# zhizdev/sparsefusion

Measured on AMD Instinct MI355X. Metric: novel views/sec, distillation steps (2 NGP renders fwd+bwd + VAE enc/dec + 51-eval PLMS + LPIPS), 256^2 / 32x32 latents, 2-view synthetic hydrant, higher is better.
Workload: dtype bf16 MFMA operands / f32 accumulate (UNet); f32 (NGP render)

## Files before the change

### include/sparsefusion_hip.h

```cpp
#ifndef SPARSEFUSION_HIP_H
#define SPARSEFUSION_HIP_H

#include <stdint.h>

#ifdef __cplusplus
extern "C" {
#endif

#define SF_OK 0
#define SF_ERR_INVALID 1
#define SF_ERR_LAUNCH 2

const char* sf_last_error(void);
int sf_abi_version(void);
int sf_operand_is_f16(void);


int sf_grid_encode_forward(const float* inputs, const float* embeddings,
                           const int32_t* offsets, float* outputs,
                           uint32_t B, uint32_t D, uint32_t C, uint32_t L,
                           float S, uint32_t H, float* dy_dx,
                           uint32_t gridtype, int align_corners,
                           const int32_t* h_offsets, void* stream);

// ... 174 lines not shown
  uint32_t n_tensors;
  float beta1, beta2, eps;
  float bias_correction2_sqrt;
  float one_minus_beta1, one_minus_beta2;
} sf_adam_args;
int sf_adam_multi(const sf_adam_args* args, void* stream);

uint32_t sf_loss_partial_rows(void);
int sf_upsample2x_forward(const float* in, float* out, uint32_t planes, uint32_t h, uint32_t w, void* stream);
int sf_upsample2x_backward(const float* grad_out, float* grad_in, uint32_t planes, uint32_t h, uint32_t w, void* stream);
int sf_render_loss_forward(const float* img, const float* sil, const float* target_rgb, const float* target_mask, uint64_t n_img,
                           uint64_t n_sil, float scaling, float* partial, void* stream);
int sf_render_loss_backward(const float* img, const float* sil, const float* target_rgb, const float* target_mask, uint64_t n_img,
                            uint64_t n_sil, float scaling, float c_rgb, float c_sil, float c_opacity, float c_entropy,
                            const float* grad_loss, float* grad_img, float* grad_sil, void* stream);
int sf_fusion_loss_forward(const float* img, const float* pred, const float* view_weight, const float* sil, uint32_t views,
                           uint64_t per_view_img, uint64_t per_view_sil, float* partial, void* stream);
int sf_fusion_loss_backward(const float* img, const float* pred, const float* view_weight, const float* sil, uint32_t views,
                            uint64_t per_view_img, uint64_t per_view_sil, float c_l1, float c_opacity, float c_entropy,
                            const float* grad_loss, float* grad_img, float* grad_sil, void* stream);

int sf_plan_run(const sf_op* ops, uint32_t n_ops, void* stream);
uint64_t sf_conv_igemm_t_launches(void);
int sf_plan_profile(const sf_op* ops, uint32_t n_ops, void* stream, float* h_ms);

uint64_t sf_conv_packed_elems(uint32_t Cout, uint32_t cin_pad, uint32_t kh, uint32_t kw);
int sf_conv_pack_weights(const float* h_w, uint32_t Cout, uint32_t Cin,
                         uint32_t cin_pad, uint32_t kh, uint32_t kw,
                         uint16_t* h_out);

int sf_plms_update(const float* x, const float* eps, const float* noise,
                   const float* h_coef6, uint64_t n, float* x_prev, float* x0,
                   void* stream);
int sf_plms_combine(const float* e0, const float* e1, const float* e2,
                    const float* e3, const float* h_c4, uint64_t n, float* out,
                    float* keep_e0, void* stream);
int sf_plms_step(const float* e0, const float* e1, const float* e2, const float* e3,
                 const float* h_c4, float* keep_e0, const float* x, const float* noise,
                 const float* h_coef6, uint64_t n, float* x_prev,
                 const float* row_src, float* row_dst, uint64_t row_n, void* stream);

#ifdef __cplusplus
}
#endif
#endif
```

### sparsefusion_amd/_lib.py

```python
import ctypes as C
import os

import torch

_HERE = os.path.dirname(os.path.abspath(__file__))
_DEFAULT_LIB = "libsparsefusion_hip_f16.so" if os.environ.get("SF_OPERAND", "bf16").lower() in ("f16", "fp16", "half") else "libsparsefusion_hip.so"
LIB_PATH = os.environ.get("SF_HIP_LIB") or os.path.join(_HERE, _DEFAULT_LIB)

_lib = None

c_f32p = C.c_void_p
c_i32p = C.c_void_p
u32 = C.c_uint32
u64 = C.c_uint64


class SfNgpField(C.Structure):
    _fields_ = [("embeddings", C.c_void_p), ("h_offsets", C.c_void_p), ("L", u32), ("S", C.c_float),
                ("H", u32), ("gridtype", u32),
                ("w0", C.c_void_p), ("b0", C.c_void_p), ("w1", C.c_void_p), ("b1", C.c_void_p),
                ("w2", C.c_void_p), ("b2", C.c_void_p), ("bound", C.c_float)]


class SfNgpFieldGrad(C.Structure):
# ... 54 lines not shown
    "sf_fusion_loss_forward": (C.c_int, [c_f32p, c_f32p, c_f32p, c_f32p, u32, u64, u64, c_f32p, C.c_void_p]),
    "sf_fusion_loss_backward": (C.c_int, [c_f32p, c_f32p, c_f32p, c_f32p, u32, u64, u64, C.c_float, C.c_float, C.c_float,
                                          c_f32p, c_f32p, c_f32p, C.c_void_p]),
    "sf_ngp_density": (C.c_int, [C.POINTER(SfNgpField), c_f32p, u32, c_f32p, c_f32p, C.c_void_p]),
    "sf_ngp_density_lattice": (C.c_int, [C.POINTER(SfNgpField), c_f32p, c_f32p, c_f32p, u32, u32, u32, c_f32p, C.c_void_p]),
    "sf_gaussian3d_workspace_bytes": (u64, [u32, u32, u32]),
    "sf_gaussian3d": (C.c_int, [c_f32p, c_f32p, u32, u32, u32, C.c_float, C.c_float, C.c_void_p, C.c_void_p, u64, C.c_void_p]),
    "sf_mc_workspace_bytes": (u64, [u32, u32, u32]),
    "sf_mc_count": (C.c_int, [c_f32p, u32, u32, u32, C.c_float, C.c_void_p, u64, C.c_void_p, C.c_void_p]),
    "sf_mc_emit": (C.c_int, [c_f32p, u32, u32, u32, C.c_float, C.c_void_p, u64, c_f32p, c_i32p, C.c_void_p]),
    "sf_ngp_render_forward": (C.c_int, [C.POINTER(SfNgpField), c_f32p, c_f32p, c_f32p, u32, u32, C.c_float,
                                        c_f32p, c_f32p, c_f32p, u32, C.c_float, c_f32p, c_f32p, c_f32p, c_f32p,
                                        c_f32p, c_f32p, c_f32p, c_f32p, c_f32p, c_f32p, u64, C.c_void_p]),
    "sf_ngp_render_backward": (C.c_int, [C.POINTER(SfNgpField), C.POINTER(SfNgpFieldGrad), c_f32p, c_f32p,
                                         c_f32p, u32, u32, c_f32p, c_f32p, c_f32p, c_f32p, c_f32p,
                                         C.c_float, c_f32p, c_f32p, u32, c_f32p, c_f32p, u64, C.c_void_p]),
    "sf_ngp_render_workspace_bytes": (u64, [u32, u32]),
    "sf_ngp_render_forward_workspace_bytes": (u64, [u32, u32]),
    "sf_ngp_render_cache_bytes": (u64, [u32, u32]),
    "sf_ngp_render_occ_eval": (C.c_int, [C.POINTER(SfNgpField), c_f32p, c_f32p, c_f32p, c_f32p, C.c_void_p, C.c_float, u32, u32, u32,
                                         c_f32p, C.c_float, u32, c_f32p, c_f32p, c_f32p, C.c_void_p]),
    "sf_plan_run": (C.c_int, [C.POINTER(SfOp), u32, C.c_void_p]),
    "sf_conv_igemm_t_launches": (u64, []),
    "sf_plan_profile": (C.c_int, [C.POINTER(SfOp), u32, C.c_void_p, C.c_void_p]),
    "sf_conv_packed_elems": (u64, [u32, u32, u32, u32]),
    "sf_conv_pack_weights": (C.c_int, [C.c_void_p, u32, u32, u32, u32, u32, C.c_void_p]),
    "sf_plms_update": (C.c_int, [c_f32p, c_f32p, c_f32p, C.c_void_p, u64, c_f32p, c_f32p, C.c_void_p]),
    "sf_plms_combine": (C.c_int, [c_f32p, c_f32p, c_f32p, c_f32p, C.c_void_p, u64, c_f32p, c_f32p, C.c_void_p]),
    "sf_plms_step": (C.c_int, [c_f32p, c_f32p, c_f32p, c_f32p, C.c_void_p, c_f32p, c_f32p, c_f32p, C.c_void_p, u64, c_f32p, c_f32p, c_f32p, u64, C.c_void_p]),
}


_handles = {}


def _load(path):
    if path not in _handles:
        if not os.path.exists(path):
            raise RuntimeError(
                f"{path} is missing: build it with `python -m sparsefusion_amd.build` (`--f16` for the IEEE-half operand build; "
                "there is no CPU fallback for the sparsefusion_amd hot path)")
        handle = C.CDLL(path)
        for name, (res, args) in SIGNATURES.items():
            fn = getattr(handle, name)
            fn.restype = res
            fn.argtypes = args
# ... 40 lines not shown
```

### sparsefusion_amd/csrc/conv_igemm_t.h

```cpp
#pragma once
#include "sf_dev.h"
#include "conv_lds.h"

#define SF_IGT_SPLITK 0
#define SF_IGT_PIXSHUF 1

#define SF_IGEMM_T_VARIANTS(X) \
  X(5, 256, 256, 4, 2, 1, 0, 2, 2, 4, 1, 0) \
  X(4, 256, 512, 4, 2, 1, 0, 1, 2, 8, 1, 0) \
  X(3, 512, 1024, 4, 2, 1, 0, 1, 1, 4, 1, 0) \
  X(2, 1024, 4096, 1, 1, 0, 0, 1, 1, 1, 1, 1) \
  X(3, 1024, 2048, 1, 1, 0, 0, 1, 1, 1, 1, 1) \
  X(4, 512, 1024, 1, 1, 0, 0, 1, 2, 1, 1, 1) \
  X(5, 256, 4, 3, 1, 1, 0, 1, 1, 4, 1, 0)

constexpr int sf_igt_log2(int v) { return v <= 1 ? 0 : 1 + sf_igt_log2(v >> 1); }

#ifndef SF_IGT_KNOCKOUT
#define SF_IGT_KNOCKOUT 0
#endif

template <int HL, int CIN, int COUT, int K, int STRIDE, int PAD, int UPS, int WM, int WN, int GROUPS, bool A_FP32, int EPI>
SF_KERNEL(256) void k_conv_igemm_t(ConvArgs a) {
  constexpr int H = 1 << HL, HO = (H + 2 * PAD - K) / STRIDE + 1, HOL = sf_igt_log2(HO), M = HO * HO;
  constexpr int CCH = CIN / 32, CCL = sf_igt_log2(CCH), KS = K * K * CCH, NF = (COUT + 15) / 16, NPAD = NF * 16;
  constexpr int MT = M / 16 / WM, NT = NF / WN, SPW = (KS + GROUPS * 4 - 1) / (GROUPS * 4);
  constexpr bool RAGGED = SPW * GROUPS * 4 != KS;
  constexpr int STEP_REGS = WM * (A_FP32 ? 8 : 4) + WN * 4;
  constexpr int D = SPW * STEP_REGS <= 96 ? SPW : (96 / STEP_REGS < 2 ? 2 : 96 / STEP_REGS);
  constexpr int LDC = COUT / 4;
  static_assert((1 << HOL) == HO && (1 << CCL) == CCH && CIN % 32 == 0, "k_conv_igemm_t: power-of-two map and channel chunks");
  static_assert(M % (16 * WM) == 0 && NF % WN == 0, "k_conv_igemm_t: the tiles divide the output evenly (no clamped fragments)");
  static_assert(EPI == SF_IGT_SPLITK ? GROUPS > 1 : (GROUPS == 1 && COUT % 64 == 0 && M % 16 == 0), "k_conv_igemm_t: epilogue kind");
  static_assert(H * H * CIN < (1 << 28) && NF * KS * 64 < (1 << 27) && GROUPS * M * NPAD < (1 << 29), "k_conv_igemm_t: 32-bit offsets");

  sf_touch_kernarg<(int)sizeof(ConvArgs)>();
  SF_SHARED __attribute__((aligned(16))) float red[3][WM * WN * 4 * 64];
  const int lane = threadIdx.x & 63, wave = sf_uniform((int)(threadIdx.x >> 6));
  const int tile = blockIdx.x % (MT * NT), grp = blockIdx.x / (MT * NT);
  const int nt = tile % NT, mt = tile / NT;
  const int k0 = (grp * 4 + wave) * SPW;
  const int cgrp = (lane >> 4) * 8;

  float bq[WN];
#pragma unroll
  for (int ni = 0; ni < WN; ++ni) bq[ni] = EPI == SF_IGT_PIXSHUF ? a.bias[(nt * WN + ni) * 16 + (lane & 15)] : 0.0f;

  int py[WM], px[WM];
#pragma unroll
  for (int mi = 0; mi < WM; ++mi) {
    const int m = (mt * WM + mi) * 16 + (lane & 15);
    py[mi] = (m >> HOL) * STRIDE - PAD;
    px[mi] = (m & (HO - 1)) * STRIDE - PAD;
  }
  const float* in32 = reinterpret_cast<const float*>(a.in);
  const sf_opnd* in16 = reinterpret_cast<const sf_opnd*>(a.in);
// ... 70 lines not shown
        for (int r = 0; r < 4; ++r) red[wave - 1][((mi * WN + ni) * 4 + r) * 64 + lane] = acc[mi][ni][r];
  }
  sf_sync();
  if (wave != 0) return;
#pragma unroll
  for (int mi = 0; mi < WM; ++mi)
#pragma unroll
    for (int ni = 0; ni < WN; ++ni)
#pragma unroll
      for (int r = 0; r < 4; ++r) {
        const int idx = ((mi * WN + ni) * 4 + r) * 64 + lane;
        acc[mi][ni][r] += red[0][idx] + red[1][idx] + red[2][idx];
      }
  if (SF_IGT_KNOCKOUT == 3) {
#ifndef SF_HOST_EMU
#pragma unroll
    for (int mi = 0; mi < WM; ++mi)
#pragma unroll
      for (int ni = 0; ni < WN; ++ni) asm volatile("" ::"v"(acc[mi][ni]), "v"(bq[ni]));
#endif
    return;
  }

#pragma unroll
  for (int mi = 0; mi < WM; ++mi) {
#pragma unroll
    for (int ni = 0; ni < WN; ++ni) {
      const int nf = nt * WN + ni;
      const int n = nf * 16 + (lane & 15);
      const int m0 = (mt * WM + mi) * 16 + (lane >> 4) * 4;
      if (EPI == SF_IGT_SPLITK) {
#pragma unroll
        for (int r = 0; r < 4; ++r) a.ws[(grp * M + m0 + r) * NPAD + n] = acc[mi][ni][r];
      } else {
        float bv = bq[ni];
        SF_USE_FROM_HERE(bv);
        float v[4], sm = 0.0f, sq = 0.0f;
#pragma unroll
        for (int r = 0; r < 4; ++r) {
          v[r] = sf_silu(acc[mi][ni][r] + bv);
          sm += v[r];
          sq = fmaf(v[r], v[r], sq);
        }
        sm = sf_wave_sum(sm);
        sq = sf_wave_sum(sq);
        if (lane == 0) {
          float* sl = a.slots_out + (((mt * WM + mi) * 4 + (nf & 3)) * (LDC >> 4) + (nf >> 2)) * 2;
          sl[0] = sm;
          sl[1] = sq;
        }
        const int c = n >> 2, ii = (n >> 1) & 1, jj = n & 1;
#pragma unroll
        for (int r = 0; r < 4; ++r) {
          const int m = m0 + r, oy = m >> HOL, ox = m & (HO - 1);
          a.out[((2 * oy + ii) * (2 * HO) + 2 * ox + jj) * LDC + c] = v[r];
        }
      }
    }
  }
}
```

### sparsefusion_amd/csrc/initx.hip

```cpp
#include "sf_common.h"
#include "initx.h"

int sf_plan_initx_op(const sf_op* op, void* stream) {
  InitXArgs a;
  a.x = (const float*)op->p[0]; a.base = (const float*)op->p[1]; a.w = (const ix_bf16x8*)op->p[2]; a.out = (float*)op->p[3];
  a.slots = (float*)op->p[4];
  a.B = op->i[0]; a.H = op->i[1]; a.W = op->i[2]; a.Cx = op->i[3]; a.ld = op->i[4];
  for (int k = 0; k < 3; ++k) { a.cw[k] = op->i[5 + k]; a.co[k] = op->i[8 + k]; a.woff[k] = op->i[11 + k]; }
  if (!a.x || !a.base || !a.w || !a.out || a.B < 1) SF_FAIL(SF_ERR_INVALID, "init_x: missing operand");
  if (a.H % IX_TILE || a.W % IX_TILE || a.Cx < 1 || a.Cx > 4) SF_FAIL(SF_ERR_INVALID, "init_x: H, W multiples of 8 and 1..4 latent channels");
  if ((a.cw[0] != 64 && a.cw[0] != 128) || (a.cw[1] != 32 && a.cw[1] != 64) || (a.cw[2] != 32 && a.cw[2] != 64))
    SF_FAIL(SF_ERR_INVALID, "init_x: channel slices (%d, %d, %d) not instantiated", a.cw[0], a.cw[1], a.cw[2]);
  if (a.slots && (a.ld % 16 || a.co[0] % 16 || a.co[1] % 16 || a.co[2] % 16)) SF_FAIL(SF_ERR_INVALID, "init_x: slots need 16-aligned channel slices");
  const uint32_t grid = (uint32_t)a.B * (a.H / IX_TILE) * (a.W / IX_TILE) * 3;
  k_init_x<<<grid, 256, 0, (hipStream_t)stream>>>(a);
  SF_CHECK_LAUNCH("init_x");
  return SF_OK;
}
```

### sparsefusion_amd/csrc/unet_ops.hip

```cpp

#include "sf_common.h"
#include "plan_ops.h"
#include "sf_dev.h"
#include "gemm_rows.h"
#include "conv_halo.h"
#include "conv_halo_small.h"
#include "conv_igemm.h"
#include "conv_igemm_t.h"
#include "attn_ln.h"
#include <math.h>

typedef __attribute__((ext_vector_type(8))) sf_opnd bf16x8;
typedef __attribute__((ext_vector_type(4))) sf_opnd bf16x4;
typedef __attribute__((ext_vector_type(4))) float f32x4;
typedef __attribute__((address_space(1))) float gfloat;

__device__ __forceinline__ void atomic_add_f32(float* p, float v) {
  (void)__builtin_amdgcn_global_atomic_fadd_f32((gfloat*)p, v);
}
__device__ __forceinline__ float silu_f(float v) { return v / (1.0f + __expf(-v)); }
__device__ __forceinline__ float sigmoid_f(float v) { return 1.0f / (1.0f + __expf(-v)); }
__device__ __forceinline__ float gelu_f(float v) { return 0.5f * v * (1.0f + erff(v * 0.70710678118654752f)); }

__device__ __forceinline__ float wave_sum(float v) {
// ... 402 lines not shown
  for (long i = blockIdx.x * 256L + threadIdx.x; i < n; i += (long)gridDim.x * 256) out[i] += a[i];
}

__global__ void k_time_emb(const float* __restrict__ t, const float* __restrict__ w, float* __restrict__ out, int B,
                           int half) {
  const int i = blockIdx.x * blockDim.x + threadIdx.x;
  if (i >= B * half) return;
  const int b = i / half, j = i - b * half;
  const float fr = t[b] * w[j] * 2.0f * 3.14159265358979323846f;
  float* o = out + (long)b * (1 + 2 * half);
  if (j == 0) o[0] = t[b];
  o[1 + j] = sinf(fr);
  o[1 + half + j] = cosf(fr);
}

template <int WM, int WN>
static void launch_conv(const ConvArgs& a, bool a_fp32, int blocks, hipStream_t st) {
  if (a_fp32) k_conv_igemm<WM, WN, true><<<blocks, 256, 0, st>>>(a);
  else k_conv_igemm<WM, WN, false><<<blocks, 256, 0, st>>>(a);
}

static unsigned long long g_igemm_t_launches = 0;
extern "C" uint64_t sf_conv_igemm_t_launches(void) { return g_igemm_t_launches; }
static bool launch_conv_t(const ConvArgs& a, int WM, int WN, bool a_fp32, int blocks, hipStream_t st) {
  if (a.B != 1 || a.H != a.W || a.kh != a.kw || a.accum || a.resid || a.relu || a.co_off) return false;
  const int epi = a.pixshuf ? SF_IGT_PIXSHUF : SF_IGT_SPLITK;
  if (a.pixshuf ? (!a.slots_out || !a.bias || a.ldc * 4 != a.Cout || a.groups != 1) : (a.groups < 2 || !a.ws)) return false;
#define SF_TRY_IGT(hl_, cin_, cout_, k_, s_, p_, ups_, wm_, wn_, g_, f32_, epi_) \
  if (a.H == (1 << hl_) && a.Cin == cin_ && a.Cout == cout_ && a.kh == k_ && a.stride == s_ && a.pad == p_ && a.ups == ups_ && WM == wm_ && \
      WN == wn_ && a.groups == g_ && a_fp32 == (bool)f32_ && epi == epi_ && a.Ho == ((1 << hl_) + 2 * p_ - k_) / s_ + 1 && a.Wo == a.Ho) { \
    k_conv_igemm_t<hl_, cin_, cout_, k_, s_, p_, ups_, wm_, wn_, g_, (bool)f32_, epi_><<<blocks, 256, 0, st>>>(a); \
    ++g_igemm_t_launches; \
    return true; \
  }
  SF_IGEMM_T_VARIANTS(SF_TRY_IGT)
#undef SF_TRY_IGT
  return false;
}

static int conv_glds_depth() { return 4; }
template <int BNF, int NST, bool GN>
static int launch_conv_glds(const ConvArgs& a, int nblk, double* part, int cg, hipStream_t st) {
  static unsigned mask = 0;
  const uint32_t lds = conv_glds_lds_bytes(BNF, NST);
  int dev = 0;
  if (hipGetDevice(&dev) != hipSuccess) SF_FAIL(SF_ERR_LAUNCH, "hipGetDevice failed");
  if (dev >= 32 || !(mask & (1u << dev))) {
    if (hipFuncSetAttribute(reinterpret_cast<const void*>(&k_conv_glds<BNF, NST, GN>), hipFuncAttributeMaxDynamicSharedMemorySize, (int)lds) != hipSuccess)
      SF_FAIL(SF_ERR_LAUNCH, "hipFuncSetAttribute(max dynamic LDS) failed");
    if (dev < 32) mask |= 1u << dev;
  }
  k_conv_glds<BNF, NST, GN><<<nblk, 512, lds, st>>>(a, part, cg);
  SF_CHECK_LAUNCH("conv_glds");
  return SF_OK;
// ... 126 lines not shown
      } else if (bnf == 4) {
        if (f32) k_conv_lds_gn<4, true><<<nblk, 256, 0, st>>>(a, part, cg); else k_conv_lds_gn<4, false><<<nblk, 256, 0, st>>>(a, part, cg);
      } else {
        SF_FAIL(SF_ERR_INVALID, "conv: unsupported LDS tile %d", bnf);
      }
      SF_CHECK_LAUNCH("conv_lds_gn");
      return SF_OK;
    }
    if (halo) return bnf == 8 ? launch_conv_halo_nst<8, false>(a, nblk, nullptr, 0, halo, st) : launch_conv_halo_nst<4, false>(a, nblk, nullptr, 0, halo, st);
    if (glds) {
      if (int rc = bnf == 8 ? launch_conv_glds_nst<8, false>(a, nblk, nullptr, 0, glds, st) : launch_conv_glds_nst<4, false>(a, nblk, nullptr, 0, glds, st)) return rc;
      return conv_splitk_tail(op, a, M, st);
    }
    if (bnf == 8) {
      if (f32) k_conv_lds<8, true><<<nblk, 256, 0, st>>>(a); else k_conv_lds<8, false><<<nblk, 256, 0, st>>>(a);
    } else if (bnf == 4) {
      if (f32) k_conv_lds<4, true><<<nblk, 256, 0, st>>>(a); else k_conv_lds<4, false><<<nblk, 256, 0, st>>>(a);
    } else {
      SF_FAIL(SF_ERR_INVALID, "conv: unsupported LDS tile %d", bnf);
    }
    SF_CHECK_LAUNCH("conv_lds");
    return conv_splitk_tail(op, a, M, st);
  }
  if ((op.flags & 512) && launch_conv_t(a, WM, WN, f32, blocks, st)) {
    SF_CHECK_LAUNCH("conv_igemm_t");
    return conv_splitk_tail(op, a, M, st);
  }
  switch (tile) {
    case 1 * 16 + 1: launch_conv<1, 1>(a, f32, blocks, st); break;
    case 1 * 16 + 2: launch_conv<1, 2>(a, f32, blocks, st); break;
    case 1 * 16 + 4: launch_conv<1, 4>(a, f32, blocks, st); break;
    case 2 * 16 + 1: launch_conv<2, 1>(a, f32, blocks, st); break;
    case 2 * 16 + 2: launch_conv<2, 2>(a, f32, blocks, st); break;
    case 2 * 16 + 4: launch_conv<2, 4>(a, f32, blocks, st); break;
    case 4 * 16 + 1: launch_conv<4, 1>(a, f32, blocks, st); break;
    case 4 * 16 + 2: launch_conv<4, 2>(a, f32, blocks, st); break;
    case 4 * 16 + 4: launch_conv<4, 4>(a, f32, blocks, st); break;
    default: SF_FAIL(SF_ERR_INVALID, "conv: unsupported wave tile %dx%d", WM, WN);
  }
  SF_CHECK_LAUNCH("conv_igemm");
  return conv_splitk_tail(op, a, M, st);
}

static int lazy_from_op(const sf_op& op, int ibase, int M, LazySrc& lz) {
  lz.mode = op.i[ibase]; lz.groups = op.i[ibase + 1]; lz.npad = op.i[ibase + 2]; lz.M = M;
  lz.a = (const float*)op.p[8]; lz.b = (const float*)op.p[9]; lz.r = (const float*)op.p[10];
  if (lz.mode < 0 || lz.mode > 2) SF_FAIL(SF_ERR_INVALID, "lazy source: unknown mode %d", lz.mode);
// ... 419 lines not shown
```

### sparsefusion_amd/plan.py

```python
import torch

from . import _lib

OP_CONV, OP_GN_ACT, OP_LN, OP_GEMV, OP_ATTN, OP_GCA_POOL, OP_ELTWISE, OP_MEMSET, OP_TIME_EMB, OP_SPLITK_REDUCE = range(1, 11)
OP_FCONV, OP_SLOTS, OP_GCA, OP_INITX, OP_GN_FINALIZE = 14, 15, 16, 17, 18
FNORM_NONE, FNORM_GN_SELF, FNORM_GN_SLOTS, FNORM_LN, FNORM_ATTN = range(5)
LDS_MAX = 163840
SKIP_SCALE = 2 ** -0.5


class _Arena:

    def __init__(self, nbytes=None, device=None):
        self.off = 0
        self.buf = torch.empty(nbytes, dtype=torch.uint8, device=device) if nbytes else None

    def alloc(self, nbytes):
        nbytes = (nbytes + 255) // 256 * 256
        off = self.off
        self.off += nbytes
        return (self.buf.data_ptr() + off) if self.buf is not None else (1 << 20) + off


class _T:
    __slots__ = ("ptr", "rows", "C", "HW", "lazy", "slots", "writer", "twin")

    def __init__(self, ptr, rows, C, HW=None):
        self.ptr, self.rows, self.C, self.HW = ptr, rows, C, HW
        self.lazy = None
        self.slots = None
        self.twin = None
        self.writer = None


class PlanOwner:
    conv_waves_target = 1024
    lds_conv_min_blocks = 0
    lds_mid_min_rows = 0
    lds_mid_min_batch = 8
    gn_epilogue = False
    gn_one = True
    ln_wave = True
    tb_stride = 0
    lazy_consumers = 0
    ss_total = 0
    igemm_t = 0
    igemm_t_variants = ()
    tile_override = None

    def conv_tiling(self, m_frags, n_frags, KS, pixshuf=False):
        ov = self.tile_override
        if ov and (m_frags, n_frags, KS, bool(pixshuf)) in ov:
            return ov[(m_frags, n_frags, KS, bool(pixshuf))]
        best = None
        mfma = m_frags * n_frags * KS
        w_bytes = n_frags * KS * 1024
        for WM in (1, 2, 4):
            if m_frags % WM or (m_frags <= 4 and WM != m_frags and m_frags in (1, 2, 4)):
                continue
            for WN in (1, 2, 4):
                if n_frags % WN:
                    continue
                tiles = (m_frags // WM) * (n_frags // WN)
                for groups in ((1,) if pixshuf else (1, 2, 4, 8, 16, 32)):
                    if groups > 1 and KS // (4 * groups) < 2:
                        continue
                    waves = tiles * groups * 4
                    util = min(1.0, waves / self.conv_waves_target)
                    t_hbm = w_bytes / 4.0e12 / util
# ... 118 lines not shown
                tile, groups = 256 + bnf, 1
                if twin is not None and ldc == Cout and co_off == 0:
                    twin_ws = twin.ptr
            elif mid and M >= mid:
                glds_ok = not x_f32 and x.C % 64 == 0 and Cout % 4 == 0 and ldc % 4 == 0 and co_off % 4 == 0
                stages = KS // 2 if glds_ok else (KS + 1) // 2
                g = 1 if pixshuf else max(1, min(256 // blocks, stages // 4, 16))
                if glds_ok and k == 3 and stride == 1 and pad == 1 and H == W and H in (4, 8) and not pixshuf:
                    g = max(1, min(256 // blocks, x.C // 128, 16))
                tile, groups = 256 + bnf, g
        ws, wi = 0, 0
        if groups > 1:
            wi = self.acquire_ws(groups * M * n_frags * 16 * 4)
            ws = self.ws_ptrs[wi]
        elif twin_ws:
            ws = twin_ws
        defer = bool(defer and not relu and not gelu and 1 < groups <= defer_max_groups and not accum and not pixshuf and co_off == 0 and ldc == Cout == out.C and M == out.rows
                     and (self.u.lazy_consumers & 1))
        bias, res = self.wptr(bname) if bname else 0, resid.ptr if resid else 0
        slots = 0
        if want_slots and pixshuf and tile < 256 and (Cout // 4) % 16 == 0 and ldc % 16 == 0 and co_off % 16 == 0 and (Ho * Wo) % 16 == 0 and not accum:
            slots = self.misc.alloc(4 * M // 16 * (ldc // 16) * 2 * 4)
        nchw = bool(nchw and groups > 1 and not defer and not accum and not resid and tile < 256 and co_off == 0 and ldc == Cout)
        igt = False
        if self.u.igemm_t and tile < 256 and B == 1 and H == W and (Ho, Wo) == ((H + 2 * pad - k) // stride + 1,) * 2 and not (accum or res or relu or gelu or co_off):
            key = (H.bit_length() - 1, x.C, Cout, k, stride, pad, int(bool(upsampled)), WM, WN, groups, int(bool(x_f32)), 1 if pixshuf else 0)
            if key in self.u.igemm_t_variants and H == 1 << key[0] and (self.u.igemm_t >> self.u.igemm_t_variants.index(key)) & 1:
                igt = bool(slots and bias and ldc * 4 == Cout) if pixshuf else groups > 1
        self.op(OP_CONV, (1 if x_f32 else 0) | (2 if pixshuf else 0) | (4 if accum else 0) | (8 if defer else 0) |
                (16 if upsampled else 0) | (32 if relu else 0) | (64 if gelu else 0) | (256 if nchw else 0) | (512 if igt else 0),
                p=(x.ptr, w_ptr if w_ptr is not None else self.wptr(wname), bias, out.ptr, res, ws, 0, slots),
                i=(B, H, W, x.C, Ho, Wo, Cout, ldc, co_off, k, k, stride, pad, groups, tile))
        if defer:
            out.lazy = ("splitk", ws, bias, res, groups, n_frags * 16, wi)
            self.ws_owners[wi] = out
        out.slots = slots or None
        self.last_conv_nchw = nchw
        out.writer = self.ops[-1] if (tile >= 256 and co_off == 0 and ldc == Cout == out.C and M == out.rows) else None
        out.twin = twin if (twin is not None and tile >= 256 and groups == 1 and ws == twin.ptr) else None
        return Ho, Wo

    def gn_act(self, x, skip, gname, ss_ptr, out, raw=None, silu=True, groups=8, eps=1e-5):
        C1, C2 = x.C, (skip.C if skip else 0)
        self.need(skip)
        lp, li = self.take_lazy(x, ("splitk", "gate"))
        stats = self.zero.alloc(self.B * groups * 2 * 8)
        ready = 0
        wr = x.writer
        cg = (C1 // groups) if not skip else 0
        if (self.u.gn_epilogue and wr is not None and not (wr.flags & 128) and li[0] == 0 and cg in (4, 8, 16)
                and x.HW and x.HW % 128 == 0 and x.rows == self.B * x.HW):
            part = self.misc.alloc(x.rows // 128 * groups * 2 * 8)
            wr.flags |= 128
# ... 43 lines not shown
```

### sparsefusion_amd/unet.py

```python
import math
import os

import numpy as np
import torch
import torch.nn as nn

from . import _lib
from .plan import (FNORM_ATTN, FNORM_GN_SELF, FNORM_GN_SLOTS, FNORM_LN, FNORM_NONE, LDS_MAX, OP_ATTN, OP_CONV, OP_ELTWISE, OP_FCONV, OP_GCA,
                   OP_GCA_POOL, OP_GEMV, OP_GN_ACT, OP_GN_FINALIZE, OP_INITX, OP_LN, OP_MEMSET, OP_SLOTS, OP_SPLITK_REDUCE, OP_TIME_EMB,
                   SKIP_SCALE, Plan, PlanOwner, _T)

PAIR_TILES = {(1, 1, 1), (1, 1, 2), (1, 2, 2), (2, 2, 2), (4, 2, 2)}
PIPE_TILES = {(1, 1, 4), (1, 2, 4), (1, 1, 6), (1, 2, 6), (2, 1, 6), (2, 2, 6), (2, 1, 8), (2, 2, 8), (2, 1, 12), (2, 2, 12), (4, 1, 16), (4, 2, 16)}
CONV3S_VARIANTS = {(5, 256, 5, 2, 2), (5, 256, 3, 2, 2), (4, 256, 4, 1, 1), (4, 256, 2, 1, 1), (4, 512, 4, 1, 2), (4, 512, 2, 1, 2),
                   (3, 512, 3, 1, 1), (3, 1024, 3, 1, 1), (5, 256, 5, 4, 2), (5, 256, 3, 4, 2),
                   (4, 256, 2, 2, 1), (4, 256, 2, 2, 2), (4, 512, 2, 2, 2), (3, 512, 3, 2, 1), (3, 1024, 3, 2, 1), (3, 1024, 3, 2, 2)}
CONV3S_RC_VARIANTS = {(5, 256, 256, 256, 3, 2, 2), (4, 512, 256, 512, 2, 1, 2), (3, 1024, 512, 1024, 3, 1, 1)}
IGEMM_T_VARIANTS = ((5, 256, 256, 4, 2, 1, 0, 2, 2, 4, 1, 0), (4, 256, 512, 4, 2, 1, 0, 1, 2, 8, 1, 0), (3, 512, 1024, 4, 2, 1, 0, 1, 1, 4, 1, 0),
                    (2, 1024, 4096, 1, 1, 0, 0, 1, 1, 1, 1, 1), (3, 1024, 2048, 1, 1, 0, 0, 1, 1, 1, 1, 1), (4, 512, 1024, 1, 1, 0, 0, 1, 2, 1, 1, 1),
                    (5, 256, 4, 3, 1, 1, 0, 1, 1, 4, 1, 0))
ATTN_LDS_BYTES = 8 * 16 * 36 * 4 + 2 * 8 * 4 * 68 * 4
TILE_PICKS = {(4, 32, 128, False): (1, 2, 8),
              (4, 128, 32, True): (1, 1, 1),
              (16, 64, 16, True): (1, 2, 1),
              (64, 1, 72, False): (1, 1, 4),
              (64, 16, 128, False): (2, 4, 4), (16, 32, 128, False): (1, 4, 4), (4, 64, 256, False): (1, 2, 4),
              (4, 64, 288, False): (1, 4, 4), (4, 256, 32, True): (1, 2, 1), (16, 128, 32, True): (1, 4, 1),
              (64, 64, 16, True): (1, 2, 1)}

SWITCHES = (
    ("conv_waves_target", 1024, "waves wanted per conv launch (4 per CU) before split-K stops"),
    ("lds_conv_min_blocks", 96, "use k_conv_lds when a layer has at least this many 128 x 128 output tiles"),
    ("lds_mid_min_rows", 128, "r06: convs of >= this many rows that have too few 128-row tiles for lds_conv_min_blocks run on the LDS-tiled kernels with split-K groups (Plan.conv); 0 = off"),
    ("igemm_t", 127, "the one-of-a-kind implicit GEMMs of the B = 1 eval on k_conv_igemm_t (compile-time geometry, csrc/conv_igemm_t.h; op flag 512): bit j = row j of IGEMM_T_VARIANTS; 0: k_conv_igemm"),
    ("merged_down_conv4", True, "r06: the merged 3x3 + 1x1 conv of the last Downsample on k_conv4_gn<64, 0, false> at B = 1; False: k_conv_igemm"),
    ("rc_small_tiles", 32, "r06: bit mask of map sides (32 | 16 | 8) whose B >= 2 (conv1 || res_conv) pairs keep the B = 1 tile of k_conv3s_rc (32: B = 2 eval 1.155 -> 1.139 ms, B = 4 1.562 -> 1.520; 32 | 16: B = 4 1.580, B = 8 2.451 -> 2.550)"),
    ("gn_one", True, "r06: GroupNorm passes of B >= 32 plans (B * 8 >= 256 workgroups) in one launch (k_gn_one); False: k_gn_stats + k_gn_apply everywhere"),
    ("lds_mid_min_batch", 8, "... in plans of at least this many images (the B = 1 .. 4 plans keep their measured kernels)"),
    ("unfused_min_rows_4", 256, "r06: 4x4-level ResnetBlocks with B*16 >= this leave the fused kernels (as unfused_min_rows at 32x32 / 16x16; measured: B = 8 loses 0.12 ms, B = 16 gains 0.22, B = 32 0.49); 0 = never"),
    ("unfused_min_rows_8", 1024, "... 8x8 level (k_conv3_halo_sm; measured: B = 8 loses 0.14 ms, B = 16 gains 0.04, B = 32 0.56)"),
    ("unfused_lin_min_rows", 256, "r06: attention / feed-forward linears of the 4x4 level with >= this many token rows leave the fused kernels (measured: B = 16 3.683 -> 3.670 ms, B = 32 4.664 -> 4.472)"),
    ("unfused_min_rows_16", 4096, "r06: the 16x16 level's own threshold (0 = unfused_min_rows; measured with k_gemm_rows_ks / the r06 plans: B = 16 3.641 -> 3.313 ms; 2048 rows lose: B = 8 2.454 -> 2.512)"),
    ("unfused_min_rows_32", 0, "... 32x32 level (4096 rows lose: B = 4 1.575 -> 1.686 ms)"),
    ("unfused_min_rows", 8192, "ResnetBlocks with B*H*W >= this at the 32x32 / 16x16 levels leave the fused kernels (_Plan.resnet; measured r03: B = 8 eval 3.33 -> 2.96 ms, B = 32 11.5 -> 7.8 ms, B = 4 unchanged)"),
    ("lazy_consumers", 3, "bit 0: split-K reductions, bit 1: gated residuals are materialised by their first consumer"),
    ("fused", True, "GroupNorm inside the conv launches (k_conv_fused) wherever the layer fits; False = the first-round plan"),
    ("pair_res_conv", True, "conv1 || res_conv of a ResnetBlock in one launch"),
    ("res_conv_beside_pool", True, "4x4 gca blocks: the res_conv shares the GlobalContext pooling launch instead"),
    ("initx_direct", True, "latent half of the init conv as one direct-convolution launch"),
    ("big_tile_min_batch", 2, "batch from which the 8x8 / 16x16 / 32x32 maps use 32- / 32- / 64-pixel tiles (r03: B = 2 eval 1.70 -> 1.50 ms, B = 4 2.62 -> 2.02, B = 32 16.4 -> 11.5; at B = 1 they would leave half the CUs idle; 999 = never)"),
    ("gca_epilogue_pool", True, "GlobalContext pooling in conv2's epilogue (False = k_gca_pool launch)"),
    ("fconv_pipe", True, "slot-GroupNorm 3x3 convs on k_conv_fused_pipe (staging || matrix work)"),
    ("producer_slots", True, "r04: k_init_x / the Upsample epilogue leave their consumers' statistics slots, the final conv's split-K reduction writes NCHW (False: the r03 k_slots / k_unpack_out launches; parity tests)"),
    ("attn_in_out_proj", True, "the 16-token attention core in the prologue of its output projection (False: k_attn16 launch; parity tests)"),
    ("ln_wave", True, "r05: LayerNorm of <= 256 rows of 512 | 1024 | 2048 channels on k_layernorm_wave (False: op flag 4 = k_layernorm)"),
    ("gate_t", True, "r05: GlobalContext gate with a compile-time hidden width (k_gca_gate_t; False: k_gca_gate)"),
    ("conv4_reduce_min_batch", 4, "r05: from this batch on a 4x4 split-K conv1 is reduced by its own launch instead of by conv2's gather (0 = never)"),
# ... 631 lines not shown
        self.x_in, self.t_in = self.f32(B, u.channels * HW), self.f32(B, 1)
        self.cond_in = self.f32(B, u.cond_images_channels * HW)
        self.tb = self.f32(B, u.tb_stride)
        self.ss = self.tb
        self.emit_time(B, self.tb.ptr, self.t_in.ptr)
        self.n_time_ops = len(self.ops)
        self.op(OP_MEMSET, 0, p=(self.zero.buf.data_ptr() if self.zero.buf is not None else 1,), i=(0,))
        memset_op = self.ops[-1]
        xin = self.f32(B * HW, cpad, HW)
        self.op(OP_ELTWISE, 2, p=(self.cond_in.ptr, self.x_in.ptr, 0, xin.ptr), i=(B, HW, u.cond_images_channels, u.channels, cpad))
        x = self.f32(B * HW, u.dim, HW)
        co = 0
        for i, k in enumerate((3, 7, 15)):
            cw = u.spec_shapes[f"init_conv.convs.{i}.weight"][0]
            self.conv(xin, True, R, R, f"init_conv.convs.{i}.weight", f"init_conv.convs.{i}.bias", x, u.dim, co, cw, k, 1, k // 2)
            co += cw
        self.n_init_ops = len(self.ops)
        self.x0, self.base = x, self.f32(B * HW, u.dim, HW)
        full_ops, full_written, self.ops, self.written = self.ops, self.written, [], set()
        cws = [u.spec_shapes[f"init_conv.convs.{i}.weight"][0] for i in range(3)]
        if (u.initx_direct and u.fused and R % 8 == 0 and u.channels <= 4 and cws[0] in (64, 128)
                and cws[1] in (32, 64) and cws[2] in (32, 64) and "__init_xw__" in self.w):
            offs, woffs = [0, cws[0], cws[0] + cws[1]], u.initx_woffs
            self.op(OP_INITX, 0, p=(self.x_in.ptr, self.base.ptr, self.wptr("__init_xw__"), x.ptr),
                    i=(B, R, R, u.channels, u.dim, cws[0], cws[1], cws[2], offs[0], offs[1], offs[2], woffs[0], woffs[1], woffs[2]))
        else:
            xin_x = self.f32(B * HW, 32, HW)
            self.op(OP_ELTWISE, 2, p=(self.x_in.ptr, self.x_in.ptr, 0, xin_x.ptr), i=(B, HW, 0, u.channels, 32))
            co = 0
            for i, k in enumerate((3, 7, 15)):
                cw = cws[i]
                self.conv(xin_x, True, R, R, f"__init_x__.{i}", None, x, u.dim, co, cw, k, 1, k // 2, resid=self.base)
                co += cw
        self.init_x_ops, self.ops, self.written = self.ops, full_ops, full_written
        hiddens = []
        H = R
        n_lv = len(u.in_out)
        for lv, (di, do) in enumerate(u.in_out):
            x = self.resnet(f"downs.{lv}.1", x, None, di, H)
            for r in range(u.nres[lv]):
                x = self.resnet(f"downs.{lv}.2.{r}", x, None, di, H, gca=True)
                hiddens.append(x)
            if u.attns[lv]:
                x = self.transformer(f"downs.{lv}.3", x)
            hiddens.append(x)
            if lv < n_lv - 1:
                y = self.f32(B * (H // 2) ** 2, do, (H // 2) ** 2)
# ... 443 lines not shown
```

Measured before the change: 17.76.

## Add compile-time-geometry init_x kernel and optional LDS-transposed pixel-shuffle epilogue

Adds k_init_x_t, a specialised kernel for the B = 1 sampler's latent init convolution (3/7/15 kernels) with weights preloaded into registers and one m-fragment per workgroup. It is enabled by default through a new op flag. It also adds an optional PIXLDS path that stages the pixel-shuffle epilogue of k_conv_igemm_t through LDS so the output goes out as vector stores; that path is off by default (pixshuf_lds = 0). The cost targeted is a small part of each UNet eval, so the effect on the whole distillation step is limited, and the heavier register use of the new kernel could lower occupancy.

New measurement: 17.83, median of 6. About the same (+0.4%).

```diff
diff --git a/include/sparsefusion_hip.h b/include/sparsefusion_hip.h
--- a/include/sparsefusion_hip.h
+++ b/include/sparsefusion_hip.h
@@ -220,6 +220,8 @@
 
 int sf_plan_run(const sf_op* ops, uint32_t n_ops, void* stream);
 uint64_t sf_conv_igemm_t_launches(void);
+uint64_t sf_conv_pixshuf_lds_launches(void);
+uint64_t sf_init_x_t_launches(void);
 int sf_plan_profile(const sf_op* ops, uint32_t n_ops, void* stream, float* h_ms);
 
 uint64_t sf_conv_packed_elems(uint32_t Cout, uint32_t cin_pad, uint32_t kh, uint32_t kw);
diff --git a/sparsefusion_amd/_lib.py b/sparsefusion_amd/_lib.py
--- a/sparsefusion_amd/_lib.py
+++ b/sparsefusion_amd/_lib.py
@@ -100,6 +100,8 @@
                                          c_f32p, C.c_float, u32, c_f32p, c_f32p, c_f32p, C.c_void_p]),
     "sf_plan_run": (C.c_int, [C.POINTER(SfOp), u32, C.c_void_p]),
     "sf_conv_igemm_t_launches": (u64, []),
+    "sf_conv_pixshuf_lds_launches": (u64, []),
+    "sf_init_x_t_launches": (u64, []),
     "sf_plan_profile": (C.c_int, [C.POINTER(SfOp), u32, C.c_void_p, C.c_void_p]),
     "sf_conv_packed_elems": (u64, [u32, u32, u32, u32]),
     "sf_conv_pack_weights": (C.c_int, [C.c_void_p, u32, u32, u32, u32, u32, C.c_void_p]),
diff --git a/sparsefusion_amd/csrc/conv_igemm_t.h b/sparsefusion_amd/csrc/conv_igemm_t.h
--- a/sparsefusion_amd/csrc/conv_igemm_t.h
+++ b/sparsefusion_amd/csrc/conv_igemm_t.h
@@ -20,7 +20,7 @@
 #define SF_IGT_KNOCKOUT 0
 #endif
 
-template <int HL, int CIN, int COUT, int K, int STRIDE, int PAD, int UPS, int WM, int WN, int GROUPS, bool A_FP32, int EPI>
+template <int HL, int CIN, int COUT, int K, int STRIDE, int PAD, int UPS, int WM, int WN, int GROUPS, bool A_FP32, int EPI, bool PIXLDS = false>
 SF_KERNEL(256) void k_conv_igemm_t(ConvArgs a) {
   constexpr int H = 1 << HL, HO = (H + 2 * PAD - K) / STRIDE + 1, HOL = sf_igt_log2(HO), M = HO * HO;
   constexpr int CCH = CIN / 32, CCL = sf_igt_log2(CCH), KS = K * K * CCH, NF = (COUT + 15) / 16, NPAD = NF * 16;
@@ -32,6 +32,7 @@
   static_assert((1 << HOL) == HO && (1 << CCL) == CCH && CIN % 32 == 0, "k_conv_igemm_t: power-of-two map and channel chunks");
   static_assert(M % (16 * WM) == 0 && NF % WN == 0, "k_conv_igemm_t: the tiles divide the output evenly (no clamped fragments)");
   static_assert(EPI == SF_IGT_SPLITK ? GROUPS > 1 : (GROUPS == 1 && COUT % 64 == 0 && M % 16 == 0), "k_conv_igemm_t: epilogue kind");
+  static_assert(!PIXLDS || EPI == SF_IGT_PIXSHUF, "k_conv_igemm_t: the LDS transpose belongs to the pixel-shuffle epilogue");
   static_assert(H * H * CIN < (1 << 28) && NF * KS * 64 < (1 << 27) && GROUPS * M * NPAD < (1 << 29), "k_conv_igemm_t: 32-bit offsets");
 
   sf_touch_kernarg<(int)sizeof(ConvArgs)>();
@@ -148,6 +149,8 @@
     return;
   }
 
+  float* tr = &red[0][0];
+  if (PIXLDS) sf_wave_sync();
 #pragma unroll
   for (int mi = 0; mi < WM; ++mi) {
 #pragma unroll
@@ -176,6 +179,11 @@
           sl[1] = sq;
         }
         const int c = n >> 2, ii = (n >> 1) & 1, jj = n & 1;
+        if (PIXLDS) {
+#pragma unroll
+          for (int r = 0; r < 4; ++r) tr[((mi * 16 + (lane >> 4) * 4 + r) * 4 + (lane & 3)) * (WN * 4) + ni * 4 + ((lane & 15) >> 2)] = v[r];
+          continue;
+        }
 #pragma unroll
         for (int r = 0; r < 4; ++r) {
           const int m = m0 + r, oy = m >> HOL, ox = m & (HO - 1);
@@ -184,4 +192,15 @@
       }
     }
   }
+  if (PIXLDS) {
+    sf_wave_sync();
+#pragma unroll
+    for (int q = 0; q < WM * WN; ++q) {
+      const int idx = q * 64 + lane;
+      const int op = idx / WN, part = idx % WN;
+      const int m = mt * WM * 16 + (op >> 2), oy = m >> HOL, ox = m & (HO - 1), ii = (op >> 1) & 1, jj = op & 1;
+      *reinterpret_cast<f32x4*>(a.out + ((2 * oy + ii) * (2 * HO) + 2 * ox + jj) * LDC + (nt * WN + part) * 4) =
+          *reinterpret_cast<const f32x4*>(tr + idx * 4);
+    }
+  }
 }
diff --git a/sparsefusion_amd/csrc/initx.hip b/sparsefusion_amd/csrc/initx.hip
--- a/sparsefusion_amd/csrc/initx.hip
+++ b/sparsefusion_amd/csrc/initx.hip
@@ -1,5 +1,9 @@
 #include "sf_common.h"
 #include "initx.h"
+#include "initx_t.h"
+
+static unsigned long long g_init_x_t_launches = 0;
+extern "C" uint64_t sf_init_x_t_launches(void) { return g_init_x_t_launches; }
 
 int sf_plan_initx_op(const sf_op* op, void* stream) {
   InitXArgs a;
@@ -12,6 +16,17 @@
   if ((a.cw[0] != 64 && a.cw[0] != 128) || (a.cw[1] != 32 && a.cw[1] != 64) || (a.cw[2] != 32 && a.cw[2] != 64))
     SF_FAIL(SF_ERR_INVALID, "init_x: channel slices (%d, %d, %d) not instantiated", a.cw[0], a.cw[1], a.cw[2]);
   if (a.slots && (a.ld % 16 || a.co[0] % 16 || a.co[1] % 16 || a.co[2] % 16)) SF_FAIL(SF_ERR_INVALID, "init_x: slots need 16-aligned channel slices");
+  if (op->flags & 1) {
+#define SF_TRY_IXT(hl_, cw0_, cw1_, cw2_) \
+    if (initx_t_matches<hl_, cw0_, cw1_, cw2_>(a)) { \
+      k_init_x_t<hl_, cw0_, cw1_, cw2_><<<3u << (2 * hl_ - 4), 256, 0, (hipStream_t)stream>>>(a); \
+      ++g_init_x_t_launches; \
+      SF_CHECK_LAUNCH("init_x_t"); \
+      return SF_OK; \
+    }
+    SF_INIT_X_T_VARIANTS(SF_TRY_IXT)
+#undef SF_TRY_IXT
+  }
   const uint32_t grid = (uint32_t)a.B * (a.H / IX_TILE) * (a.W / IX_TILE) * 3;
   k_init_x<<<grid, 256, 0, (hipStream_t)stream>>>(a);
   SF_CHECK_LAUNCH("init_x");
diff --git a/sparsefusion_amd/csrc/initx_t.h b/sparsefusion_amd/csrc/initx_t.h
--- /dev/null
+++ b/sparsefusion_amd/csrc/initx_t.h
@@ -0,0 +1,125 @@
+#pragma once
+#include "initx.h"
+
+#define SF_INIT_X_T_VARIANTS(X) \
+  X(5, 128, 64, 64)
+
+#define IXT_PATCH_BYTES (16 * 24 * 8 + 16)
+
+template <int HL, int CW0, int CW1, int CW2>
+inline bool initx_t_matches(const InitXArgs& a) {
+  return a.B == 1 && a.H == (1 << HL) && a.W == (1 << HL) && a.Cx == 4 && a.ld == CW0 + CW1 + CW2 && a.cw[0] == CW0 && a.cw[1] == CW1 &&
+         a.cw[2] == CW2 && a.co[0] == 0 && a.co[1] == CW0 && a.co[2] == CW0 + CW1 && a.woff[0] == 0 && a.woff[1] == 2 * (CW0 / 16) &&
+         a.woff[2] == 2 * (CW0 / 16) + 7 * (CW1 / 16);
+}
+
+template <int HL, int LD, int K, int CW, int CO, int WOFF>
+SF_DEV void initx_t_conv(const InitXArgs& a, char* __restrict__ patch, int tid, int f) {
+  constexpr int H = 1 << HL, HALO = K / 2;
+  constexpr int STEPS = K == 15 ? 30 : (K == 7 ? 7 : 2);
+  constexpr int NF = CW / 16, NFW = NF / 4;
+  constexpr int PH = K == 3 ? 5 : 2 + 2 * HALO;
+  constexpr int PW = K == 15 ? 24 : (K == 7 ? 16 : 12);
+  constexpr int PWV = K == 15 ? 22 : PW;
+  constexpr int RL = K == 7 ? 4 : 5;
+  constexpr int IT = ((PH << RL) + 255) / 256;
+  static_assert(NF % 4 == 0 && PW <= (1 << RL) && (PH * PW + 1) * 8 <= IXT_PATCH_BYTES && LD % 16 == 0 && CO % 16 == 0, "k_init_x_t: geometry");
+  const int lane = tid & 63, wave = sf_uniform(tid >> 6);
+  const int n = lane & 15, g = lane >> 4;
+  const int y0 = ((f >> (HL - 1)) << 3) + ((f & 3) << 1);
+  const int x0 = ((f >> 2) & ((H >> 3) - 1)) << 3;
+
+  float v[IT][4];
+  bool in[IT];
+#pragma unroll
+  for (int it = 0; it < IT; ++it) {
+    const int i = tid + it * 256;
+    const int fy = i >> RL, fx = i & ((1 << RL) - 1);
+    const int yy = y0 - HALO + fy, xx = x0 - HALO + fx;
+    in[it] = fx < PWV && (unsigned)yy < (unsigned)H && (unsigned)xx < (unsigned)H;
+    const int yc = min(max(yy, 0), H - 1), xc = min(max(xx, 0), H - 1);
+#pragma unroll
+    for (int c = 0; c < 4; ++c) v[it][c] = a.x[(((c << HL) + yc) << HL) + xc];
+  }
+  const ix_bf16x8* __restrict__ w = a.w + WOFF * 64 + lane;
+  ix_bf16x8 wf[STEPS][NFW];
+#pragma unroll
+  for (int s = 0; s < STEPS; ++s)
+#pragma unroll
+    for (int j = 0; j < NFW; ++j) wf[s][j] = w[(s * NF + wave + 4 * j) * 64];
+  const int m0 = ((y0 + (g >> 1)) << HL) + x0 + ((g & 1) << 2);
+  const int c0 = m0 * LD + CO + wave * 16 + n;
+  float bv[4][NFW];
+#pragma unroll
+  for (int r = 0; r < 4; ++r)
+#pragma unroll
+    for (int j = 0; j < NFW; ++j) bv[r][j] = a.base[c0 + r * LD + j * 64];
+
+#pragma unroll
+  for (int it = 0; it < IT; ++it) {
+    const int i = tid + it * 256;
+    const int fy = i >> RL, fx = i & ((1 << RL) - 1);
+    ix_bf16x4 o;
+#pragma unroll
+    for (int c = 0; c < 4; ++c) o[c] = (sf_opnd)(in[it] ? v[it][c] : 0.0f);
+    *reinterpret_cast<ix_bf16x4*>(patch + ((fy < PH && fx < PW) ? fy * PW + fx : PH * PW) * 8) = o;
+  }
+  sf_sync();
+
+  ix_f32x4 acc[NFW];
+#pragma unroll
+  for (int j = 0; j < NFW; ++j) acc[j] = ix_f32x4{0.f, 0.f, 0.f, 0.f};
+  const int y = (lane >> 3) & 1, x = lane & 7;
+  constexpr int NH = K == 15 ? 2 : 1;
+  const int lrow = K == 3 ? (g >> 1) : 0;
+  const int lcol = K == 3 ? (g & 1) * 2 : 2 * g;
+  const char* pa0 = patch + ((y + lrow) * PW + x + lcol) * 8;
+#pragma unroll
+  for (int st = 0; st < STEPS; ++st) {
+    const int row = K == 3 ? 2 * st : st / NH, h = st % NH;
+    const char* pa = pa0 + (row * PW + h * 8) * 8;
+    const ix_bf16x4 lo = *reinterpret_cast<const ix_bf16x4*>(pa), hi = *reinterpret_cast<const ix_bf16x4*>(pa + 8);
+    const ix_bf16x8 fa = __builtin_shufflevector(lo, hi, 0, 1, 2, 3, 4, 5, 6, 7);
+#pragma unroll
+    for (int j = 0; j < NFW; ++j) acc[j] = sf_mfma16(fa, wf[st][j], acc[j]);
+  }
+
+  float sm[NFW], sq[NFW];
+#pragma unroll
+  for (int j = 0; j < NFW; ++j) sm[j] = sq[j] = 0.0f;
+#pragma unroll
+  for (int r = 0; r < 4; ++r)
+#pragma unroll
+    for (int j = 0; j < NFW; ++j) {
+      float b = bv[r][j];
+      SF_USE_FROM_HERE(b);
+      const float o = b + acc[j][r];
+      a.out[c0 + r * LD + j * 64] = o;
+      sm[j] += o;
+      sq[j] = fmaf(o, o, sq[j]);
+    }
+  if (a.slots) {
+#pragma unroll
+    for (int j = 0; j < NFW; ++j) {
+      const float s1 = sf_wave_sum(sm[j]), s2 = sf_wave_sum(sq[j]);
+      if (lane == 0) {
+        float* sl = a.slots + ((f * (LD >> 4) + (CO >> 4) + wave + 4 * j) << 1);
+        sl[0] = s1;
+        sl[1] = s2;
+      }
+    }
+  }
+}
+
+template <int HL, int CW0, int CW1, int CW2>
+SF_KERNEL(256) void k_init_x_t(InitXArgs a) {
+  constexpr int MF = (1 << (2 * HL)) >> 4, LD = CW0 + CW1 + CW2;
+  static_assert(HL >= 3 && HL <= 8, "k_init_x_t: whole 8 x 8 tiles, 32-bit offsets");
+  sf_touch_kernarg<(int)sizeof(InitXArgs)>();
+  SF_SHARED __attribute__((aligned(16))) char patch[IXT_PATCH_BYTES];
+  const int tid = threadIdx.x;
+  const int part = sf_uniform((int)blockIdx.x / MF), f = sf_uniform((int)blockIdx.x % MF);
+  if (part == 0) initx_t_conv<HL, LD, 15, CW2, CW0 + CW1, 2 * (CW0 / 16) + 7 * (CW1 / 16)>(a, patch, tid, f);
+  else if (part == 1) initx_t_conv<HL, LD, 7, CW1, CW0, 2 * (CW0 / 16)>(a, patch, tid, f);
+  else initx_t_conv<HL, LD, 3, CW0, 0, 0>(a, patch, tid, f);
+}
diff --git a/sparsefusion_amd/csrc/unet_ops.hip b/sparsefusion_amd/csrc/unet_ops.hip
--- a/sparsefusion_amd/csrc/unet_ops.hip
+++ b/sparsefusion_amd/csrc/unet_ops.hip
@@ -448,14 +448,21 @@
 
 static unsigned long long g_igemm_t_launches = 0;
 extern "C" uint64_t sf_conv_igemm_t_launches(void) { return g_igemm_t_launches; }
-static bool launch_conv_t(const ConvArgs& a, int WM, int WN, bool a_fp32, int blocks, hipStream_t st) {
+static unsigned long long g_pixshuf_lds_launches = 0;
+extern "C" uint64_t sf_conv_pixshuf_lds_launches(void) { return g_pixshuf_lds_launches; }
+static bool launch_conv_t(const ConvArgs& a, int WM, int WN, bool a_fp32, bool pix_lds, int blocks, hipStream_t st) {
   if (a.B != 1 || a.H != a.W || a.kh != a.kw || a.accum || a.resid || a.relu || a.co_off) return false;
   const int epi = a.pixshuf ? SF_IGT_PIXSHUF : SF_IGT_SPLITK;
   if (a.pixshuf ? (!a.slots_out || !a.bias || a.ldc * 4 != a.Cout || a.groups != 1) : (a.groups < 2 || !a.ws)) return false;
 #define SF_TRY_IGT(hl_, cin_, cout_, k_, s_, p_, ups_, wm_, wn_, g_, f32_, epi_) \
   if (a.H == (1 << hl_) && a.Cin == cin_ && a.Cout == cout_ && a.kh == k_ && a.stride == s_ && a.pad == p_ && a.ups == ups_ && WM == wm_ && \
       WN == wn_ && a.groups == g_ && a_fp32 == (bool)f32_ && epi == epi_ && a.Ho == ((1 << hl_) + 2 * p_ - k_) / s_ + 1 && a.Wo == a.Ho) { \
-    k_conv_igemm_t<hl_, cin_, cout_, k_, s_, p_, ups_, wm_, wn_, g_, (bool)f32_, epi_><<<blocks, 256, 0, st>>>(a); \
+    if (pix_lds && epi_ == SF_IGT_PIXSHUF) { \
+      k_conv_igemm_t<hl_, cin_, cout_, k_, s_, p_, ups_, wm_, wn_, g_, (bool)f32_, epi_, epi_ == SF_IGT_PIXSHUF><<<blocks, 256, 0, st>>>(a); \
+      ++g_pixshuf_lds_launches; \
+    } else { \
+      k_conv_igemm_t<hl_, cin_, cout_, k_, s_, p_, ups_, wm_, wn_, g_, (bool)f32_, epi_><<<blocks, 256, 0, st>>>(a); \
+    } \
     ++g_igemm_t_launches; \
     return true; \
   }
@@ -628,7 +635,7 @@
     SF_CHECK_LAUNCH("conv_lds");
     return conv_splitk_tail(op, a, M, st);
   }
-  if ((op.flags & 512) && launch_conv_t(a, WM, WN, f32, blocks, st)) {
+  if ((op.flags & 512) && launch_conv_t(a, WM, WN, f32, (op.flags & 1024) != 0, blocks, st)) {
     SF_CHECK_LAUNCH("conv_igemm_t");
     return conv_splitk_tail(op, a, M, st);
   }
diff --git a/sparsefusion_amd/plan.py b/sparsefusion_amd/plan.py
--- a/sparsefusion_amd/plan.py
+++ b/sparsefusion_amd/plan.py
@@ -45,6 +45,7 @@
     lazy_consumers = 0
     ss_total = 0
     igemm_t = 0
+    pixshuf_lds = 0
     igemm_t_variants = ()
     tile_override = None
 
@@ -209,13 +210,16 @@
         if want_slots and pixshuf and tile < 256 and (Cout // 4) % 16 == 0 and ldc % 16 == 0 and co_off % 16 == 0 and (Ho * Wo) % 16 == 0 and not accum:
             slots = self.misc.alloc(4 * M // 16 * (ldc // 16) * 2 * 4)
         nchw = bool(nchw and groups > 1 and not defer and not accum and not resid and tile < 256 and co_off == 0 and ldc == Cout)
-        igt = False
-        if self.u.igemm_t and tile < 256 and B == 1 and H == W and (Ho, Wo) == ((H + 2 * pad - k) // stride + 1,) * 2 and not (accum or res or relu or gelu or co_off):
+        igt, pix_lds = False, False
+        if (self.u.igemm_t or self.u.pixshuf_lds) and tile < 256 and B == 1 and H == W and (Ho, Wo) == ((H + 2 * pad - k) // stride + 1,) * 2 and not (accum or res or relu or gelu or co_off):
             key = (H.bit_length() - 1, x.C, Cout, k, stride, pad, int(bool(upsampled)), WM, WN, groups, int(bool(x_f32)), 1 if pixshuf else 0)
-            if key in self.u.igemm_t_variants and H == 1 << key[0] and (self.u.igemm_t >> self.u.igemm_t_variants.index(key)) & 1:
-                igt = bool(slots and bias and ldc * 4 == Cout) if pixshuf else groups > 1
+            if key in self.u.igemm_t_variants and H == 1 << key[0]:
+                row = self.u.igemm_t_variants.index(key)
+                ok = bool(slots and bias and ldc * 4 == Cout) if pixshuf else groups > 1
+                igt = bool(ok and (self.u.igemm_t >> row) & 1)
+                pix_lds = bool(ok and pixshuf and (self.u.pixshuf_lds >> row) & 1)
         self.op(OP_CONV, (1 if x_f32 else 0) | (2 if pixshuf else 0) | (4 if accum else 0) | (8 if defer else 0) |
-                (16 if upsampled else 0) | (32 if relu else 0) | (64 if gelu else 0) | (256 if nchw else 0) | (512 if igt else 0),
+                (16 if upsampled else 0) | (32 if relu else 0) | (64 if gelu else 0) | (256 if nchw else 0) | (512 if igt else 0) | (1024 if pix_lds else 0),
                 p=(x.ptr, w_ptr if w_ptr is not None else self.wptr(wname), bias, out.ptr, res, ws, 0, slots),
                 i=(B, H, W, x.C, Ho, Wo, Cout, ldc, co_off, k, k, stride, pad, groups, tile))
         if defer:
diff --git a/sparsefusion_amd/unet.py b/sparsefusion_amd/unet.py
--- a/sparsefusion_amd/unet.py
+++ b/sparsefusion_amd/unet.py
@@ -19,6 +19,7 @@
 IGEMM_T_VARIANTS = ((5, 256, 256, 4, 2, 1, 0, 2, 2, 4, 1, 0), (4, 256, 512, 4, 2, 1, 0, 1, 2, 8, 1, 0), (3, 512, 1024, 4, 2, 1, 0, 1, 1, 4, 1, 0),
                     (2, 1024, 4096, 1, 1, 0, 0, 1, 1, 1, 1, 1), (3, 1024, 2048, 1, 1, 0, 0, 1, 1, 1, 1, 1), (4, 512, 1024, 1, 1, 0, 0, 1, 2, 1, 1, 1),
                     (5, 256, 4, 3, 1, 1, 0, 1, 1, 4, 1, 0))
+INIT_X_T_VARIANTS = ((5, 128, 64, 64),)
 ATTN_LDS_BYTES = 8 * 16 * 36 * 4 + 2 * 8 * 4 * 68 * 4
 TILE_PICKS = {(4, 32, 128, False): (1, 2, 8),
               (4, 128, 32, True): (1, 1, 1),
@@ -33,6 +34,8 @@
     ("lds_conv_min_blocks", 96, "use k_conv_lds when a layer has at least this many 128 x 128 output tiles"),
     ("lds_mid_min_rows", 128, "r06: convs of >= this many rows that have too few 128-row tiles for lds_conv_min_blocks run on the LDS-tiled kernels with split-K groups (Plan.conv); 0 = off"),
     ("igemm_t", 127, "the one-of-a-kind implicit GEMMs of the B = 1 eval on k_conv_igemm_t (compile-time geometry, csrc/conv_igemm_t.h; op flag 512): bit j = row j of IGEMM_T_VARIANTS; 0: k_conv_igemm"),
+    ("pixshuf_lds", 0, "the PixelShuffle epilogue of k_conv_igemm_t stores through the reduction LDS (op flag 1024; csrc/conv_igemm_t.h PIXLDS): bit j = row j of IGEMM_T_VARIANTS (pixel-shuffle rows only: 56 = all three); 0: four dword stores per lane.  Off until its A/B (tools/initx_t_ab.py) is on record: DESIGN 4.10"),
+    ("init_x_t", True, "the sampler's latent init conv of the canonical B = 1 eval on k_init_x_t (compile-time geometry, one m-fragment per workgroup, csrc/initx_t.h; SF_OP_INITX flag 1); False: k_init_x"),
     ("merged_down_conv4", True, "r06: the merged 3x3 + 1x1 conv of the last Downsample on k_conv4_gn<64, 0, false> at B = 1; False: k_conv_igemm"),
     ("rc_small_tiles", 32, "r06: bit mask of map sides (32 | 16 | 8) whose B >= 2 (conv1 || res_conv) pairs keep the B = 1 tile of k_conv3s_rc (32: B = 2 eval 1.155 -> 1.139 ms, B = 4 1.562 -> 1.520; 32 | 16: B = 4 1.580, B = 8 2.451 -> 2.550)"),
     ("gn_one", True, "r06: GroupNorm passes of B >= 32 plans (B * 8 >= 256 workgroups) in one launch (k_gn_one); False: k_gn_stats + k_gn_apply everywhere"),
@@ -710,7 +713,8 @@
         if (u.initx_direct and u.fused and R % 8 == 0 and u.channels <= 4 and cws[0] in (64, 128)
                 and cws[1] in (32, 64) and cws[2] in (32, 64) and "__init_xw__" in self.w):
             offs, woffs = [0, cws[0], cws[0] + cws[1]], u.initx_woffs
-            self.op(OP_INITX, 0, p=(self.x_in.ptr, self.base.ptr, self.wptr("__init_xw__"), x.ptr),
+            ixt = bool(u.init_x_t and B == 1 and u.channels == 4 and (R.bit_length() - 1, *cws) in INIT_X_T_VARIANTS and R == 1 << (R.bit_length() - 1))
+            self.op(OP_INITX, 1 if ixt else 0, p=(self.x_in.ptr, self.base.ptr, self.wptr("__init_xw__"), x.ptr),
                     i=(B, R, R, u.channels, u.dim, cws[0], cws[1], cws[2], offs[0], offs[1], offs[2], woffs[0], woffs[1], woffs[2]))
         else:
             xin_x = self.f32(B * HW, 32, HW)
```
